# rare-resilience-ai/Osteosarcoma_DiffusionModel

Hardware: AMD Instinct MI355X
Metric: synthetic patients/sec (full T-step reverse sample) (higher is better)
Workload: dtype f32; 1 GPU; reverse sampling of conditional patients, T=1000, D=2000 (50 mut + 1900 expr + 50 pathway), hidden [256,512,256], 3 scenario conditions (BASELINE config 3); patients_per_gpu=100000, T=1000, parallelism=patients sharded over 1 GPU(s), no collective, sampler=chain, chunk_rows=65536, streams=2, graph=True

## Files before the change

osteosarcoma_diffusionmodel_amd/csrc/chain.h:

```cpp
#pragma once
#include "gemm_glds.h"
#include "epilogues.h"
#include "xpose.h"
#include "launch.h"

namespace osd {

constexpr int CHAIN_MAX_LAYERS = 24;
enum : int { CK_INPUT = 0, CK_GN32 = 1, CK_GN64 = 2, CK_POST = 3 };
enum : unsigned { CHAIN_OK = 0, CHAIN_TIMEOUT = 1, CHAIN_ABORT = 2 };

struct ChainLayer {
  const float* A; int lda;
  int K, K0;
  int F;
  int in0, ld0, in1, ld1;
  int out, ldo;
  int kind;
  const float* bias; const float* gamma; const float* beta;
};

struct ChainArgs {
  ChainLayer L[CHAIN_MAX_LAYERS];
  int n_layers;
  float* ws; long long ws_stride;
  float* x; int D;
  int n, n_tiles;
  int t_first, n_steps;
  unsigned base_done;
  const float* cproj; int ldc;
  const float* temb; int ldt;
  const float* coef;
  const float* z; int ldzz; long long z_step_stride; int z_t_first;
  uint64_t seed; uint32_t row_offset;
  float* mut_mask; int mutation_dim;
  unsigned* progress;
  unsigned* status;
  unsigned* queue;
  unsigned* cu_arrivals;
  int stagger;
  unsigned long long spin_budget;
  unsigned long long* stamps;
};

typedef __attribute__((address_space(1))) unsigned gu32;

__device__ __forceinline__ unsigned ld_relaxed_agent(const unsigned* p) {
  return __hip_atomic_load(p, __ATOMIC_RELAXED, __HIP_MEMORY_SCOPE_AGENT);
}
__device__ __forceinline__ void st_relaxed_agent(unsigned* p, unsigned v) {
  __hip_atomic_store(p, v, __ATOMIC_RELAXED, __HIP_MEMORY_SCOPE_AGENT);
}

__device__ __forceinline__ bool chain_wait(const unsigned* word, unsigned want, unsigned* status, unsigned long long budget, int lane) {
  if ((unsigned)__builtin_amdgcn_readfirstlane((int)ld_relaxed_agent(word)) >= want) return true;
  const unsigned long long t0 = __builtin_amdgcn_s_memrealtime();
  for (;;) {
    __builtin_amdgcn_s_sleep(32);
    if ((unsigned)__builtin_amdgcn_readfirstlane((int)ld_relaxed_agent(word)) >= want) return true;
    if ((unsigned)__builtin_amdgcn_readfirstlane((int)ld_relaxed_agent(status)) != CHAIN_OK) return false;
    if (__builtin_amdgcn_s_memrealtime() - t0 > budget) {
      if (lane == 0) st_relaxed_agent(status, CHAIN_TIMEOUT);
      return false;
    }
  }
}

constexpr int CHAIN_PRM_FLOATS = 512;

template <int NPB>
struct XposeRowsOut {
  const WaveXpose<NPB>& xp; float* out; int ldo;
  __device__ __forceinline__ void put(int fb, int pb, int q, int l31, int h, float4 v) const { (void)fb; xp.put(pb, q, l31, h, v); }
  __device__ __forceinline__ void flush(int fb, int lane) const { xp.template store_rows<false>(out + 32 * fb, ldo, lane, 0, 0); }
};
template <int NPB>
struct XposeRowsIn {
  const WaveXpose<NPB>& xp; const float* src; int ld;
  __device__ __forceinline__ void load(int fb, int lane) const { xp.template load_rows<false>(src + 32 * fb, ld, lane, 0, 0); }
  __device__ __forceinline__ float4 get(int fb, int pb, int q, int l31, int h) const { (void)fb; return xp.get(pb, q, l31, h); }
};

template <int GW, int NFB, int NPB, int PS, class Out>
__device__ __forceinline__ void chain_gn_silu(f32x16 (&acc)[NFB][NPB], const float* __restrict__ prm, int fl, const Out& o, int lane,
                                              unsigned long long* ts = nullptr) {
  static_assert(GW >= 8 && NFB * 32 >= GW, "wave must own whole groups");
  constexpr int RPG = GW / 2;
  constexpr int NG = NFB * 16 / RPG;
  const int l31 = lane & 31, h = lane >> 5;
#pragma unroll
  for (int fb = 0; fb < NFB; ++fb)
#pragma unroll
    for (int q = 0; q < 4; ++q) {
      const float4 bv = *reinterpret_cast<const float4*>(prm + fl + 32 * fb + 8 * q + 4 * h);
#pragma unroll
      for (int pb = 0; pb < NPB; ++pb) {
        acc[fb][pb][4 * q] += bv.x; acc[fb][pb][4 * q + 1] += bv.y;
        acc[fb][pb][4 * q + 2] += bv.z; acc[fb][pb][4 * q + 3] += bv.w;
      }
    }
  if (ts) { asm volatile("s_waitcnt vmcnt(0) lgkmcnt(0)" ::: "memory"); ts[0] = __builtin_amdgcn_s_memtime(); }
  float mean[NPB][NG], rstd[NPB][NG];
#pragma unroll
  for (int pb = 0; pb < NPB; ++pb)
#pragma unroll
    for (int g = 0; g < NG; ++g) {
      float s = 0.f;
#pragma unroll
      for (int j = 0; j < RPG; ++j) { const int Li = g * RPG + j; s += acc[Li / 16][pb][Li % 16]; }
      s += swap_halves(s);
      const float m = s * (1.0f / GW);
      float qs = 0.f;
#pragma unroll
      for (int j = 0; j < RPG; ++j) { const int Li = g * RPG + j; const float d = acc[Li / 16][pb][Li % 16] - m; qs = fmaf(d, d, qs); }
      qs += swap_halves(qs);
      mean[pb][g] = m;
      rstd[pb][g] = 1.0f / sqrtf(qs * (1.0f / GW) + GN_EPS);
    }
  if (ts) { asm volatile("s_nop 0" ::: "memory"); ts[1] = __builtin_amdgcn_s_memtime(); ts[2] = ts[1]; }
#pragma unroll
  for (int fb = 0; fb < NFB; ++fb) {
#pragma unroll
    for (int q = 0; q < 4; ++q) {
      const int f = fl + 32 * fb + 8 * q + 4 * h;
      const float4 gv = *reinterpret_cast<const float4*>(prm + PS + f);
      const float4 bev = *reinterpret_cast<const float4*>(prm + 2 * PS + f);
      const int g = (fb * 16 + 4 * q) / RPG;
#pragma unroll
      for (int pb = 0; pb < NPB; ++pb) {
        const float m = mean[pb][g], r = rstd[pb][g];
        float4 y;
        y.x = silu_f(fmaf((acc[fb][pb][4 * q] - m) * r, gv.x, bev.x));
        y.y = silu_f(fmaf((acc[fb][pb][4 * q + 1] - m) * r, gv.y, bev.y));
        y.z = silu_f(fmaf((acc[fb][pb][4 * q + 2] - m) * r, gv.z, bev.z));
        y.w = silu_f(fmaf((acc[fb][pb][4 * q + 3] - m) * r, gv.w, bev.w));
        o.put(fb, pb, q, l31, h, y);
      }
    }
    o.flush(fb, lane);
  }
}

template <int NFB, int NPB, int PS, class In, class Out>
__device__ __forceinline__ void chain_input(f32x16 (&acc)[NFB][NPB], const float* __restrict__ prm, int fl, const In& in, const Out& o, int lane) {
  const int l31 = lane & 31, h = lane >> 5;
#pragma unroll
  for (int fb = 0; fb < NFB; ++fb) {
    in.load(fb, lane);
#pragma unroll
    for (int q = 0; q < 4; ++q) {
      const int f = fl + 32 * fb + 8 * q + 4 * h;
      const float4 bv = *reinterpret_cast<const float4*>(prm + f);
      const float4 tv = *reinterpret_cast<const float4*>(prm + PS + f);
#pragma unroll
      for (int pb = 0; pb < NPB; ++pb) {
        const float4 cv = in.get(fb, pb, q, l31, h);
        float4 v;
        v.x = ((acc[fb][pb][4 * q] + bv.x) + tv.x) + cv.x;
        v.y = ((acc[fb][pb][4 * q + 1] + bv.y) + tv.y) + cv.y;
        v.z = ((acc[fb][pb][4 * q + 2] + bv.z) + tv.z) + cv.z;
        v.w = ((acc[fb][pb][4 * q + 3] + bv.w) + tv.w) + cv.w;
        o.put(fb, pb, q, l31, h, v);
      }
    }
    o.flush(fb, lane);
  }
}

#ifndef OSD_EXP
#define OSD_EXP 0
#endif
template <int NFB, int NPB, bool PRE = false, bool GUARD = true>
__device__ __forceinline__ void chain_posterior(f32x16 (&acc)[NFB][NPB], const float* __restrict__ prm, int fl, float* __restrict__ x, int ldx,
                                                int prow, int pcol, float cA, float cB, float cC, int t, const float* __restrict__ zrow, int ldzz,
                                                uint64_t seed, uint32_t row_id0, int f_glob, float* __restrict__ mut_mask, int mutation_dim,
                                                const WaveXpose<NPB>& xp, int lane, float4 (*pre)[4 * NPB] = nullptr) {
  const int l31 = lane & 31, h = lane >> 5;
  if (prow <= 0) return;
  const bool do_mask = t == 0 && mut_mask != nullptr;
#pragma unroll
  for (int fb = 0; fb < NFB; ++fb) {
    const int cols = pcol - 32 * fb;
    if (GUARD && cols <= 0) break;
    if constexpr (PRE) {
      if (!(OSD_EXP & 2)) {
        xp.commit_rows(*pre, lane);
        if (fb + 1 < NFB && cols - 32 > 0) xp.template issue_rows<GUARD>(*pre, x + 32 * (fb + 1), ldx, lane, prow, cols - 32);
      }
    } else {
      xp.template load_rows<GUARD>(x + 32 * fb, ldx, lane, prow, cols);
    }
#pragma unroll
    for (int pb = 0; pb < NPB; ++pb) {
      const int p = 32 * pb + l31;
      const int pc = (!GUARD || p < prow) ? p : prow - 1;
#pragma unroll
      for (int q = 0; q < 4; ++q) {
        const int fo = 32 * fb + 8 * q + 4 * h;
        const float4 bv = *reinterpret_cast<const float4*>(prm + fl + fo);
        const float e[4] = {acc[fb][pb][4 * q] + bv.x, acc[fb][pb][4 * q + 1] + bv.y, acc[fb][pb][4 * q + 2] + bv.z, acc[fb][pb][4 * q + 3] + bv.w};
        const float4 xq = xp.get(pb, q, l31, h);
        const float xv[4] = {xq.x, xq.y, xq.z, xq.w};
        float4 zz = make_float4(0.f, 0.f, 0.f, 0.f);
        if (t > 0 && cC != 0.f) {
          if (zrow) {
            const int fc = (!GUARD || fo < pcol - 4) ? fo : pcol - 4;
            zz = ldg4(zrow + (size_t)pc * ldzz + fc);
          } else if (!(OSD_EXP & 1)) {
            zz = randn4(seed, row_id0 + (uint32_t)p, (uint32_t)((f_glob + fo) >> 2), (uint32_t)t, TAG_POSTERIOR);
          }
        }
        const float zv[4] = {zz.x, zz.y, zz.z, zz.w};
        float o[4];
#pragma unroll
        for (int r = 0; r < 4; ++r) o[r] = fmaf(cA, xv[r], fmaf(cB, e[r], cC * zv[r]));
        if (do_mask && p < prow && fo < pcol && f_glob + fo < mutation_dim) {
          float* mrow = mut_mask + (size_t)p * mutation_dim;
#pragma unroll
          for (int r = 0; r < 4; ++r)
            if (f_glob + fo + r < mutation_dim) stg1(mrow + f_glob + fo + r, (o[r] > 0.5f) ? 1.0f : 0.0f);
        }
        xp.put(pb, q, l31, h, make_float4(o[0], o[1], o[2], o[3]));
      }
    }
    if (!(OSD_EXP & 4)) xp.template store_rows<GUARD>(x + 32 * fb, ldx, lane, prow, cols);
  }
}

#ifndef CHAIN_EPI_PRIO
#define CHAIN_EPI_PRIO 0
#endif
#ifndef CHAIN_BP
#define CHAIN_BP 128
#endif
#if CHAIN_BP == 128
typedef Tile<128, 128, 64, 64> ChainTile;
constexpr int CHAIN_WPS = 2;
#else
typedef Tile<128, 64, 64, 32> ChainTile;
constexpr int CHAIN_WPS = 3;
#endif
#ifdef OSD_DIAG
constexpr int CHAIN_KCNT = 12;
constexpr int CHAIN_STAMP_FLOATS = 2 * 4 * CHAIN_KCNT;
#else
constexpr int CHAIN_KCNT = 10;
constexpr int CHAIN_STAMP_FLOATS = 80;
#endif
constexpr int CHAIN_PRM_OFF = 2 * (ChainTile::BF * BK + ChainTile::BP * BK) + 4 + CHAIN_STAMP_FLOATS;
constexpr int CHAIN_LDS_BYTES = (CHAIN_PRM_OFF + 2 * CHAIN_PRM_FLOATS) * 4;
static_assert(CHAIN_PRM_OFF % 4 == 0, "parameter blocks are read as float4");

template <bool STAMP>
__global__ __launch_bounds__(NTHREADS, CHAIN_WPS) void chain_kernel(const ChainArgs* __restrict__ gp) {
  const ChainArgs& a = *gp;
  typedef ChainTile T;
  typedef GldsTile<T> G;
  static_assert(T::BF == 128 && T::BP % 32 == 0, "staging below assumes a 128-row weight image");
  constexpr int NW = NTHREADS / 64;
  constexpr int NPW = 16 / NW;
  constexpr int NPWB = T::BP / 8 / NW;
  constexpr int PROWS = 8 * NW;
  constexpr unsigned PBYTES = 1024u * NW;
  extern __shared__ __attribute__((aligned(16))) float smem[];
  float* As0 = smem;
  float* As1 = smem + G::A_ELEMS;
  float* Bs0 = smem + 2 * G::A_ELEMS;
  float* Bs1 = smem + 2 * G::A_ELEMS + G::B_ELEMS;
  volatile int& s_flag = *reinterpret_cast<volatile int*>(smem + 2 * (G::A_ELEMS + G::B_ELEMS));

  const int tid = threadIdx.x;
  const int lane = tid & 63;
  const int wave = __builtin_amdgcn_readfirstlane(tid >> 6);
  const int wf = (wave / T::NWP) * T::WF;
  const int wp = (wave % T::NWP) * T::WP;

  float* const ws = a.ws + (long long)blockIdx.x * a.ws_stride;
  WaveXpose<T::NPB> xp;
  {
    const int xo = wave * (T::NPB * 1024);
    xp.buf = xo < G::A_ELEMS ? As1 + xo : Bs1 + (xo - G::A_ELEMS);
  }
  float* const prm_base = smem + CHAIN_PRM_OFF;
  int pcur = 0;

  if (a.cu_arrivals && a.stagger > 0) {
    if (wave == 0) {
      const unsigned hw = __builtin_amdgcn_s_getreg(0xF804);
      const unsigned xcc = __builtin_amdgcn_s_getreg(0xF814) & 7;
      const unsigned key = (xcc << 8) | ((hw >> 8) & 0xFF);
      unsigned r = 0;
      if (lane == 0) r = atomicAdd(a.cu_arrivals + key, 1u);
      s_flag = __builtin_amdgcn_readfirstlane((int)(r & 1u));
    }
    __syncthreads();
    const int late = __builtin_amdgcn_readfirstlane(s_flag);
    __syncthreads();
    if (late) {
      const unsigned long long t0 = __builtin_amdgcn_s_memtime();
      while (__builtin_amdgcn_s_memtime() - t0 < (unsigned long long)a.stagger) __builtin_amdgcn_s_sleep(16);
    }
  }

  unsigned long long c_dep = 0, c_pro = 0, c_k = 0, c_epi = 0, c_units = 0;
  unsigned long long* const kcnt = reinterpret_cast<unsigned long long*>(smem + 2 * (G::A_ELEMS + G::B_ELEMS) + 4);
  if constexpr (STAMP) {
    if (tid < 4 * CHAIN_KCNT) kcnt[tid] = 0;
    __syncthreads();
  }
  const unsigned long long c_start = STAMP ? __builtin_amdgcn_s_memtime() : 0;
  const long long n_units = (long long)a.n_tiles * a.n_steps;
  int c_iter = 0;
  (void)c_iter;
  for (;;) {
    const unsigned long long td0 = STAMP ? __builtin_amdgcn_s_memtime() : 0;
#ifdef CHAIN_STATIC_UNITS
    static_assert(true, "");
    const long long u = (long long)blockIdx.x + (long long)c_iter * gridDim.x;
    ++c_iter;
#else
    if (wave == 0) {
      unsigned nu = 0;
      if (lane == 0) nu = atomicAdd(a.queue, 1u);
      s_flag = __builtin_amdgcn_readfirstlane((int)nu);
    }
    __syncthreads();
    const long long u = (unsigned)__builtin_amdgcn_readfirstlane(s_flag);
    __syncthreads();
#endif
    if (u >= n_units) break;
    const int tile = (int)(u % a.n_tiles);
    const int si = (int)(u / a.n_tiles);
    const int t = a.t_first - si;
    const int p0 = tile * T::BP;
    const int P = (a.n - p0 < T::BP) ? a.n - p0 : T::BP;

    if (wave == 0) {
      bool ok = (unsigned)__builtin_amdgcn_readfirstlane((int)ld_relaxed_agent(a.status)) == CHAIN_OK;
      if (ok && si > 0) {
        ok = chain_wait(a.progress + tile, a.base_done + (unsigned)si, a.status, a.spin_budget, lane);
        if (ok) __builtin_amdgcn_fence(__ATOMIC_ACQUIRE, "agent");
      }
      s_flag = ok ? 1 : 0;
      asm volatile("s_waitcnt vmcnt(0) lgkmcnt(0)" ::: "memory");
    }
    __syncthreads();
    const int go = __builtin_amdgcn_readfirstlane(s_flag);
    if (!go) return;
    if constexpr (STAMP) { c_dep += __builtin_amdgcn_s_memtime() - td0; ++c_units; }

    auto first_stage = [&](const ChainLayer& Lr, int f0n, bool do_a, bool do_b, int pb) {
      struct { const float* A; int lda, F, in0, ld0, K0, K; } Ln{Lr.A, Lr.lda, Lr.F, Lr.in0, Lr.ld0, Lr.K0, Lr.K};
      if (do_a && wave < 2) {
        const int kind = Lr.kind;
        const float* src = Lr.bias;
        if (wave == 1) src = Lr.beta;
        else if (lane >= 32) src = kind == CK_INPUT ? a.temb + (size_t)t * a.ldt : (kind == CK_POST ? Lr.bias : Lr.gamma);
        if (wave == 0 || (kind != CK_INPUT && kind != CK_POST)) {
          int f = f0n + 4 * (lane & 31);
          f = f < Ln.F - 4 ? f : Ln.F - 4;
          glds16(src + f, __builtin_amdgcn_readfirstlane(lds_addr(prm_base + pb * CHAIN_PRM_FLOATS) + (unsigned)wave * 1024u));
        }
      }
      const float* const xrows = a.x + (size_t)p0 * a.D;
      int ln = lane;
      asm volatile("" : "+v"(ln));
      const int r0 = wave * 8 + (ln >> 3);
      const int k4 = 4 * ((ln & 7) ^ ((r0 >> 1) & 7));
      const unsigned la = __builtin_amdgcn_readfirstlane(lds_addr(As0) + (unsigned)wave * 1024u);
      const unsigned lb = __builtin_amdgcn_readfirstlane(lds_addr(Bs0) + (unsigned)wave * 1024u);
      if (do_a) {
#pragma unroll
        for (int j = 0; j < NPW; ++j) {
          int rg = f0n + r0 + PROWS * j;
          rg = rg < Ln.F ? rg : Ln.F - 1;
          glds16(Ln.A + (size_t)rg * Ln.lda + k4, __builtin_amdgcn_readfirstlane(la + (unsigned)j * PBYTES));
        }
      }
      if (do_b) {
        const bool from_x = Ln.in0 < 0;
        const float* bb = from_x ? xrows : ws + Ln.in0;
        const int rows = from_x ? P : T::BP;
        const int kend = Ln.K0 < Ln.K ? Ln.K0 : Ln.K;
        const int k = k4 < kend - 4 ? k4 : kend - 4;
#pragma unroll
        for (int j = 0; j < NPWB; ++j) {
          int rg = r0 + PROWS * j;
          rg = rg < rows ? rg : rows - 1;
          glds16(bb + (size_t)rg * Ln.ld0 + k, __builtin_amdgcn_readfirstlane(lb + (unsigned)j * PBYTES));
        }
      }
    };
    unsigned long long tt0 = STAMP ? __builtin_amdgcn_s_memtime() : 0;
    first_stage(a.L[0], 0, true, true, pcur);
    asm volatile("s_waitcnt vmcnt(0)" ::: "memory");
    __syncthreads();

    for (int l = 0; l < a.n_layers; ++l) {
      const ChainLayer& L = a.L[l];
      const gfloat_ptr LA = uniform_ptr(L.A);
      const int Llda = L.lda, LK0 = L.K0, Lld0 = L.ld0, Lld1 = L.ld1;
      const int F = L.F, K = L.K;
      const float* const B0g = (L.in0 < 0) ? a.x + (size_t)p0 * a.D : ws + L.in0;
      const float* const B1g = ws + L.in1;
      const gfloat_ptr B0 = uniform_ptr(B0g), B1 = uniform_ptr(B1g);
      const int rowsB = (L.in0 < 0) ? P : T::BP;
      const int nk = (K + BK - 1) / BK;
      const int nft = (F + T::BF - 1) / T::BF;
      for (int ft = 0; ft < nft; ++ft) {
        const int f0 = ft * T::BF;
        int ln = lane;
        asm volatile("" : "+v"(ln));
        const int l31 = ln & 31, h = ln >> 5;
        int st_row[NPW], st_k4[NPW];
#pragma unroll
        for (int j = 0; j < NPW; ++j) {
          st_row[j] = (j * NW + wave) * 8 + (ln >> 3);
          st_k4[j] = 4 * ((ln & 7) ^ ((st_row[j] >> 1) & 7));
        }
        int a_rd[T::NFB], a_sw[T::NFB], b_rd[T::NPB], b_sw[T::NPB];
#pragma unroll
        for (int fb = 0; fb < T::NFB; ++fb) { const int R = wf + 32 * fb + l31; a_rd[fb] = R * BK; a_sw[fb] = h ^ ((R >> 1) & 7); }
#pragma unroll
        for (int pb = 0; pb < T::NPB; ++pb) { const int R = wp + 32 * pb + l31; b_rd[pb] = R * BK; b_sw[pb] = h ^ ((R >> 1) & 7); }
        unsigned offA[NPW], offB[NPWB];
#pragma unroll
        for (int j = 0; j < NPW; ++j) {
          int rg = f0 + st_row[j];
          rg = rg < F ? rg : F - 1;
          offA[j] = (unsigned)(rg * Llda + st_k4[j]) * 4u;
        }
#pragma unroll
        for (int j = 0; j < NPWB; ++j) {
          int rb = st_row[j];
          rb = rb < rowsB ? rb : rowsB - 1;
          offB[j] = (unsigned)(rb * Lld0 + st_k4[j]) * 4u;
        }
        int b_panel = 0;
        auto b_offsets_for = [&](int k0) {
          const int want = k0 < LK0 ? 0 : 1;
          if (want != b_panel) {
            b_panel = want;
            const int ld = want ? Lld1 : Lld0;
#pragma unroll
            for (int j = 0; j < NPWB; ++j) {
              int rb = st_row[j];
              rb = rb < rowsB ? rb : rowsB - 1;
              offB[j] = (unsigned)(rb * ld + st_k4[j]) * 4u;
            }
          }
        };
        struct StageCtx { gfloat_ptr sa, sb; unsigned la, lb; int k0; bool tail; };
        auto stage_begin = [&](int k0, float* As, float* Bs) {
          b_offsets_for(k0);
          const bool first = k0 < LK0;
          const int kend = first ? (LK0 < K ? LK0 : K) : K - LK0;
          const int kl = first ? k0 : k0 - LK0;
          StageCtx c;
          c.sa = LA + __builtin_amdgcn_readfirstlane(k0);
          c.sb = (first ? B0 : B1) + __builtin_amdgcn_readfirstlane(kl);
          c.la = __builtin_amdgcn_readfirstlane(lds_addr(As) + (unsigned)wave * 1024u);
          c.lb = __builtin_amdgcn_readfirstlane(lds_addr(Bs) + (unsigned)wave * 1024u);
          c.k0 = k0;
          c.tail = kl + BK > kend;
          return c;
        };
        auto piece = [&](const StageCtx& c, int j) {
          if (j < NPW) glds16s(c.sa, offA[j], __builtin_amdgcn_readfirstlane(c.la + (unsigned)j * PBYTES));
          else glds16s(c.sb, offB[j - NPW], __builtin_amdgcn_readfirstlane(c.lb + (unsigned)(j - NPW) * PBYTES));
        };
        auto stage_tail = [&](const StageCtx& c) {
#pragma unroll
          for (int j = 0; j < NPW; ++j) piece(c, j);
          const bool first = c.k0 < LK0;
          const int kend = first ? (LK0 < K ? LK0 : K) : K - LK0;
          const int kl = first ? c.k0 : c.k0 - LK0;
          const float* bb = first ? B0g : B1g;
          const int ld = first ? Lld0 : Lld1;
#pragma unroll
          for (int jb = 0; jb < NPWB; ++jb) {
            int k = kl + st_k4[jb];
            k = k < kend - 4 ? k : kend - 4;
            int rg = st_row[jb];
            rg = rg < rowsB ? rg : rowsB - 1;
            glds16(bb + (size_t)rg * ld + k, __builtin_amdgcn_readfirstlane(c.lb + (unsigned)jb * PBYTES));
          }
        };
        const unsigned long long tt1 = STAMP ? __builtin_amdgcn_s_memtime() : 0;

        unsigned long long c_kw = 0, c_kb = 0;
        (void)c_kw; (void)c_kb;
        f32x16 acc[T::NFB][T::NPB];
#pragma unroll
        for (int i = 0; i < T::NFB; ++i)
#pragma unroll
          for (int j = 0; j < T::NPB; ++j)
#pragma unroll
            for (int r = 0; r < 16; ++r) acc[i][j][r] = 0.f;

        float fa0[T::NFB][4], fb0[T::NPB][4], fa1[T::NFB][4], fb1[T::NPB][4];
        auto frags = [&](const float* Ac, const float* Bc, int i, float (&fa)[T::NFB][4], float (&fb)[T::NPB][4]) {
#pragma unroll
          for (int fb_ = 0; fb_ < T::NFB; ++fb_) {
            const float4 tq = *reinterpret_cast<const float4*>(&Ac[a_rd[fb_] + 4 * (a_sw[fb_] ^ (2 * i))]);
            fa[fb_][0] = tq.x; fa[fb_][1] = tq.y; fa[fb_][2] = tq.z; fa[fb_][3] = tq.w;
          }
#pragma unroll
          for (int pb = 0; pb < T::NPB; ++pb) {
            const float4 tq = *reinterpret_cast<const float4*>(&Bc[b_rd[pb] + 4 * (b_sw[pb] ^ (2 * i))]);
            fb[pb][0] = tq.x; fb[pb][1] = tq.y; fb[pb][2] = tq.z; fb[pb][3] = tq.w;
          }
        };
        auto quarter = [&](const float (&fa)[T::NFB][4], const float (&fb)[T::NPB][4]) {
#pragma unroll
          for (int e = 0; e < 4; ++e)
#pragma unroll
            for (int fb_ = 0; fb_ < T::NFB; ++fb_)
#pragma unroll
              for (int pb = 0; pb < T::NPB; ++pb)
                acc[fb_][pb] = __builtin_amdgcn_mfma_f32_32x32x2f32(fa[fb_][e], fb[pb][e], acc[fb_][pb], 0, 0, 0);
        };
        __builtin_amdgcn_sched_barrier(0);
        if (nk > 1) {
          const StageCtx c = stage_begin(BK, As1, Bs1);
          if (c.tail) stage_tail(c);
          else {
#pragma unroll
            for (int j = 0; j < NPW + NPWB; ++j) piece(c, j);
          }
        }
        frags(As0, Bs0, 0, fa0, fb0);
        __builtin_amdgcn_sched_barrier(0);
        for (int kt = 0; kt < nk; ++kt) {
          float* Ac = (kt & 1) ? As1 : As0;
          float* Bc = (kt & 1) ? Bs1 : Bs0;
          const float* An = (kt & 1) ? As0 : As1;
          const float* Bn = (kt & 1) ? Bs0 : Bs1;
          frags(Ac, Bc, 1, fa1, fb1);
          quarter(fa0, fb0);
          frags(Ac, Bc, 2, fa0, fb0);
          quarter(fa1, fb1);
          frags(Ac, Bc, 3, fa1, fb1);
          const bool ahead = kt + 2 < nk;
          StageCtx c{};
          if (ahead) c = stage_begin((kt + 2) * BK, Ac, Bc);
          const bool whole = ahead && !c.tail;
          quarter(fa0, fb0);
          __builtin_amdgcn_sched_barrier(0);
          const unsigned long long tw0 = STAMP ? __builtin_amdgcn_s_memtime() : 0;
          asm volatile("s_waitcnt vmcnt(0)" ::: "memory");
          const unsigned long long tw1 = STAMP ? __builtin_amdgcn_s_memtime() : 0;
          asm volatile("s_waitcnt lgkmcnt(0)" ::: "memory");
          __syncthreads();
          if constexpr (STAMP) { const unsigned long long tw2 = __builtin_amdgcn_s_memtime(); c_kw += tw1 - tw0; c_kb += tw2 - tw1; }
          __builtin_amdgcn_sched_barrier(0);
          if (ahead && c.tail) stage_tail(c);
          if (whole) {
#pragma unroll
            for (int j = 0; j < NPW + NPWB; ++j) piece(c, j);
          }
          if (kt + 1 < nk) frags(An, Bn, 0, fa0, fb0);
          __builtin_amdgcn_sched_barrier(0);
          quarter(fa1, fb1);
        }

        const unsigned long long tt2 = STAMP ? __builtin_amdgcn_s_memtime() : 0;
        const bool same_layer = ft + 1 < nft;
        const bool has_next = same_layer || l + 1 < a.n_layers;
        const int ln_next = same_layer ? l : l + 1;
        const int f0_next = same_layer ? f0 + T::BF : 0;
        const bool early_b = same_layer;
        if (has_next) first_stage(a.L[ln_next], f0_next, true, early_b, pcur ^ 1);
        const int fw = f0 + wf;
        const float* const prm = prm_base + pcur * CHAIN_PRM_FLOATS;
        pcur ^= 1;
        if (CHAIN_EPI_PRIO) __builtin_amdgcn_s_setprio(CHAIN_EPI_PRIO);
        const ChainArgs* ep = gp;
        asm volatile("" : "+s"(ep));
        const ChainArgs& e = *ep;
        unsigned long long ets[3] = {0, 0, 0};
        if (L.kind == CK_GN64) {
          const XposeRowsOut<T::NPB> o{xp, ws + L.out + (size_t)wp * L.ldo + fw, L.ldo};
          chain_gn_silu<64, T::NFB, T::NPB, 128>(acc, prm, wf, o, lane, STAMP ? ets : nullptr);
        } else if (L.kind == CK_GN32) {
          const XposeRowsOut<T::NPB> o{xp, ws + L.out + (size_t)wp * L.ldo + fw, L.ldo};
          chain_gn_silu<32, T::NFB, T::NPB, 128>(acc, prm, wf, o, lane, STAMP ? ets : nullptr);
        } else if (L.kind == CK_INPUT) {
          const XposeRowsIn<T::NPB> ci{xp, e.cproj + (size_t)(p0 + wp) * e.ldc + fw, e.ldc};
          const XposeRowsOut<T::NPB> o{xp, ws + L.out + (size_t)wp * L.ldo + fw, L.ldo};
          chain_input<T::NFB, T::NPB, 128>(acc, prm, wf, ci, o, lane);
        } else {
          const float* c = e.coef + 4 * t;
          const float cA = c[0], cB = c[1], cC = c[2];
          const float* zrow = e.z ? e.z + (long long)(e.z_t_first - t) * e.z_step_stride + (size_t)(p0 + wp) * e.ldzz + fw : nullptr;
          float* const mm = e.mut_mask ? e.mut_mask + (size_t)(p0 + wp) * e.mutation_dim : nullptr;
          chain_posterior<T::NFB, T::NPB>(acc, prm, wf, e.x + (size_t)(p0 + wp) * e.D + fw, e.D, P - wp, F - fw, cA, cB, cC, t, zrow, e.ldzz,
                                          e.seed, e.row_offset + (uint32_t)(p0 + wp), fw, mm, e.mutation_dim, xp, lane);
        }
        if (CHAIN_EPI_PRIO) __builtin_amdgcn_s_setprio(0);
        unsigned long long tt3 = 0, te1 = 0, te2 = 0, te3 = 0, te4 = 0;
        if constexpr (STAMP) te1 = __builtin_amdgcn_s_memtime();
        if (early_b) {
          if constexpr (STAMP) tt3 = __builtin_amdgcn_s_memtime();
          static_assert(4 * T::NFB * T::NPB == 16 || 4 * T::NFB * T::NPB == 8, "counted wait below is written for 16 or 8 stores");
          if (L.kind == CK_POST) asm volatile("s_waitcnt vmcnt(0)" ::: "memory");
          else if (4 * T::NFB * T::NPB == 16) asm volatile("s_waitcnt vmcnt(16)" ::: "memory");
          else asm volatile("s_waitcnt vmcnt(8)" ::: "memory");
          if constexpr (STAMP) te2 = __builtin_amdgcn_s_memtime();
          __syncthreads();
          if constexpr (STAMP) te3 = te4 = __builtin_amdgcn_s_memtime();
        } else {
          asm volatile("s_waitcnt vmcnt(0)" ::: "memory");
          if constexpr (STAMP) te2 = __builtin_amdgcn_s_memtime();
          __syncthreads();
          if constexpr (STAMP) tt3 = te3 = __builtin_amdgcn_s_memtime();
          if (has_next) {
            first_stage(a.L[ln_next], 0, false, true, 0);
            asm volatile("s_waitcnt vmcnt(0)" ::: "memory");
            __syncthreads();
          }
          if constexpr (STAMP) te4 = __builtin_amdgcn_s_memtime();
        }
        if constexpr (STAMP) {
          c_pro += tt1 - tt0; c_k += tt2 - tt1; c_epi += tt3 - tt2;
          tt0 = tt3;
          if (tid == 0) {
            unsigned long long* kc = kcnt + CHAIN_KCNT * L.kind;
            kc[0] += tt2 - tt1; kc[1] += te1 - tt2; kc[2] += te2 - te1; kc[3] += te3 - te2; kc[4] += te4 - te3; kc[5] += 1;
            if constexpr (CHAIN_KCNT >= 12) { kc[10] += c_kw; kc[11] += c_kb; }
            if (ets[0]) { kc[6] += ets[0] - tt2; kc[7] += ets[1] - ets[0]; kc[8] += ets[2] - ets[1]; kc[9] += te1 - ets[2]; }
          }
        }
      }
    }

    if (wave == 0) {
      __builtin_amdgcn_fence(__ATOMIC_RELEASE, "agent");
      asm volatile("s_waitcnt vmcnt(0)" ::: "memory");
      if (lane == 0) st_relaxed_agent(a.progress + tile, a.base_done + (unsigned)si + 1u);
    }
  }
  if (STAMP && a.stamps && tid == 0) {
    unsigned long long* o = a.stamps + (size_t)blockIdx.x * 64;
    o[0] = c_dep; o[1] = c_pro; o[2] = c_k; o[3] = c_epi; o[4] = __builtin_amdgcn_s_memtime() - c_start; o[5] = c_units;
    o[6] = __builtin_amdgcn_s_getreg(0xF804);
    o[7] = __builtin_amdgcn_s_getreg(0xF814) & 7;
    for (int i = 0; i < 4 * CHAIN_KCNT; ++i) o[8 + i] = kcnt[i];
  }
}

}
```

osteosarcoma_diffusionmodel_amd/csrc/gemm_glds.h:

```cpp
#pragma once
#include "gemm.h"

namespace osd {

typedef __attribute__((address_space(3))) void* lds_ptr_t;
typedef const __attribute__((address_space(1))) void* glb_ptr_t;

__device__ __forceinline__ void glds16(const float* gsrc, unsigned lds_dst) {
  unsigned keep;
  asm volatile(
      "s_mov_b32 %0, m0\n\t"
      "s_mov_b32 m0, %2\n\t"
      "s_nop 0\n\t"
      "global_load_lds_dwordx4 %1, off\n\t"
      "s_mov_b32 m0, %0"
      : "=&s"(keep)
      : "v"(gsrc), "s"(lds_dst)
      : "memory");
}
typedef const __attribute__((address_space(1))) float* gfloat_ptr;
__device__ __forceinline__ gfloat_ptr uniform_ptr(const float* p) {
  const gfloat_ptr q = (gfloat_ptr)p;
  const unsigned long long v = reinterpret_cast<unsigned long long>(q);
  const unsigned lo = __builtin_amdgcn_readfirstlane((unsigned)v), hi = __builtin_amdgcn_readfirstlane((unsigned)(v >> 32));
  return reinterpret_cast<gfloat_ptr>(((unsigned long long)hi << 32) | lo);
}
__device__ __forceinline__ void glds16s(gfloat_ptr sbase, unsigned voff, unsigned lds_dst) {
  unsigned keep;
  asm volatile(
      "s_mov_b32 %0, m0\n\t"
      "s_mov_b32 m0, %3\n\t"
      "s_nop 4\n\t"
      "global_load_lds_dwordx4 %1, %2\n\t"
      "s_mov_b32 m0, %0"
      : "=&s"(keep)
      : "v"(voff), "s"(sbase), "s"(lds_dst)
      : "memory");
}
__device__ __forceinline__ unsigned lds_addr(const float* p) {
  return (unsigned)(uintptr_t)(__attribute__((address_space(3))) const void*)p;
}

template <class T>
struct GldsTile {
  static constexpr int A_ELEMS = T::BF * BK;
  static constexpr int B_ELEMS = T::BP * BK;
  static constexpr int LDS_BYTES = 2 * (A_ELEMS + B_ELEMS) * 4;
  static constexpr int NA = T::BF / 32;
  static constexpr int NB = T::BP / 32;
};

template <class T, class Epi, int NG = 1>
__global__ __launch_bounds__(NTHREADS * NG, NG == 1 ? 2 : 1) void gemm_glds_kernel(GemmArgs g, typename Epi::Args ea) {
  typedef GldsTile<T> G;
  static_assert(NG == 1 || NG == 2, "one or two wave groups");
  extern __shared__ __attribute__((aligned(16))) float smem_all[];
  const int grp = NG == 1 ? 0 : __builtin_amdgcn_readfirstlane((int)(threadIdx.x >> 8));
  float* const smem = smem_all + grp * (G::LDS_BYTES / 4);
  float* As0 = smem;
  float* As1 = smem + G::A_ELEMS;
  float* Bs0 = smem + 2 * G::A_ELEMS;
  float* Bs1 = smem + 2 * G::A_ELEMS + G::B_ELEMS;

  const int nft = (g.F + T::BF - 1) / T::BF;
  const int npt = (g.P + T::BP - 1) / T::BP;
  const int b = blockIdx.x;
  const int idx = b >> 3;
  const int ft = idx % nft;
  int pt, pstride;
  if (g.persist) {
    const int per_xcd = gridDim.x >> 3;
    pt = idx / nft + (per_xcd / nft) * (b & 7);
    pstride = gridDim.x / nft;
  } else {
    pt = (idx / nft) * 8 + (b & 7);
    pstride = npt;
  }
  if (pt >= npt) return;
  if (g.tri && ft > pt) return;
  const int f0 = ft * T::BF;

  const int tid = threadIdx.x & (NTHREADS - 1);
  const int lane = tid & 63;
  const int wave = __builtin_amdgcn_readfirstlane(tid >> 6);
  unsigned long long st0 = 0, st1 = 0, st2 = 0;
  if (g.stamps) st0 = __builtin_amdgcn_s_memtime();
  const int wf = (wave / T::NWP) * T::WF;
  const int wp = (wave % T::NWP) * T::WP;
  const int l31 = lane & 31, h = lane >> 5;

  const auto pre = Epi::template prefetch<T::NFB, true>(ea, f0 + wf, lane, g.F);

  int a_off[G::NA], a_k4[G::NA];
  int b_k4[G::NB], b_lrow[G::NB];
#pragma unroll
  for (int j = 0; j < G::NA; ++j) {
    const int row = (j * 4 + wave) * 8 + (lane >> 3);
    int rg = f0 + row;
    rg = rg < g.F ? rg : g.F - 1;
    a_k4[j] = 4 * ((lane & 7) ^ ((row >> 1) & 7));
    a_off[j] = rg * g.lda + a_k4[j];
  }
#pragma unroll
  for (int j = 0; j < G::NB; ++j) {
    const int row = (j * 4 + wave) * 8 + (lane >> 3);
    b_lrow[j] = row;
    b_k4[j] = 4 * ((lane & 7) ^ ((row >> 1) & 7));
  }
  struct StageCtx { unsigned la, lb; const float* bbase; int bld, bk, bkend, ak, p0; };
  auto stage_begin = [&](int k0, int p0, float* As, float* Bs) {
    StageCtx c;
    c.la = __builtin_amdgcn_readfirstlane(lds_addr(As) + (unsigned)wave * 1024u);
    c.lb = __builtin_amdgcn_readfirstlane(lds_addr(Bs) + (unsigned)wave * 1024u);
    const bool first = k0 < g.K0;
    c.bbase = first ? g.B0 : g.B1;
    c.bld = first ? g.ldb0 : g.ldb1;
    c.bk = first ? k0 : k0 - g.K0;
    c.bkend = first ? (g.K0 < g.K ? g.K0 : g.K) : g.K - g.K0;
    c.ak = k0;
    c.p0 = p0;
    return c;
  };
  auto stage_piece = [&](const StageCtx& c, int j) {
    if (j < G::NA) {
      int adj = 0;
      if (g.a_kmax > 0) {
        const int k = c.ak + a_k4[j];
        adj = k < g.a_kmax - 4 ? 0 : g.a_kmax - 4 - k;
      }
      glds16(g.A + (size_t)(a_off[j] + c.ak + adj), __builtin_amdgcn_readfirstlane(c.la + (unsigned)j * 4096u));
    } else {
      const int jb = j - G::NA;
      int k = c.bk + b_k4[jb];
      k = k < c.bkend - 4 ? k : c.bkend - 4;
      int rg = c.p0 + b_lrow[jb];
      rg = rg < g.P ? rg : g.P - 1;
      glds16(c.bbase + (size_t)rg * c.bld + k, __builtin_amdgcn_readfirstlane(c.lb + (unsigned)jb * 4096u));
    }
  };
  constexpr int NPIECE = G::NA + G::NB;

  int a_rd[T::NFB], a_sw[T::NFB], b_rd[T::NPB], b_sw[T::NPB];
#pragma unroll
  for (int fb = 0; fb < T::NFB; ++fb) { const int R = wf + 32 * fb + l31; a_rd[fb] = R * BK; a_sw[fb] = h ^ ((R >> 1) & 7); }
#pragma unroll
  for (int pb = 0; pb < T::NPB; ++pb) { const int R = wp + 32 * pb + l31; b_rd[pb] = R * BK; b_sw[pb] = h ^ ((R >> 1) & 7); }

  f32x16 acc[T::NFB][T::NPB];

  auto compute = [&](const float* As, const float* Bs, int i, const StageCtx& sc, bool do_stage) {
    float a[T::NFB][4], bb[T::NPB][4];
#pragma unroll
    for (int fb = 0; fb < T::NFB; ++fb) {
      const float4 t = *reinterpret_cast<const float4*>(&As[a_rd[fb] + 4 * (a_sw[fb] ^ (2 * i))]);
      a[fb][0] = t.x; a[fb][1] = t.y; a[fb][2] = t.z; a[fb][3] = t.w;
    }
#pragma unroll
    for (int pb = 0; pb < T::NPB; ++pb) {
      const float4 t = *reinterpret_cast<const float4*>(&Bs[b_rd[pb] + 4 * (b_sw[pb] ^ (2 * i))]);
      bb[pb][0] = t.x; bb[pb][1] = t.y; bb[pb][2] = t.z; bb[pb][3] = t.w;
    }
#pragma unroll
    for (int e = 0; e < 4; ++e) {
#pragma unroll
      for (int fb = 0; fb < T::NFB; ++fb)
#pragma unroll
        for (int pb = 0; pb < T::NPB; ++pb)
          acc[fb][pb] = __builtin_amdgcn_mfma_f32_32x32x2f32(a[fb][e], bb[pb][e], acc[fb][pb], 0, 0, 0);
      if (do_stage && i == 0) {
        __builtin_amdgcn_sched_barrier(0);
        if (2 * e < NPIECE) stage_piece(sc, 2 * e);
        if (2 * e + 1 < NPIECE) stage_piece(sc, 2 * e + 1);
        __builtin_amdgcn_sched_barrier(0);
      }
    }
  };

  const int nk_all = (g.K + BK - 1) / BK;
  const int nk = NG == 1 ? nk_all : (nk_all + 1) / 2;
  const int kbeg = grp ? nk : 0;
  const int kcnt = NG == 1 ? nk : (grp ? nk_all - nk : nk);
  {
    const StageCtx c0 = stage_begin(kbeg * BK, pt * T::BP, As0, Bs0);
#pragma unroll
    for (int j = 0; j < NPIECE; ++j) stage_piece(c0, j);
  }
  constexpr int FULL_TILE_STORES = T::NFB * T::NPB * 4;
  bool counted_wait = false;
  for (; pt < npt; pt += pstride) {
    const int p0 = pt * T::BP;
    if (counted_wait) {
      if constexpr (FULL_TILE_STORES == 16) asm volatile("s_waitcnt vmcnt(16)" ::: "memory");
      else if constexpr (FULL_TILE_STORES == 8) asm volatile("s_waitcnt vmcnt(8)" ::: "memory");
      else if constexpr (FULL_TILE_STORES == 4) asm volatile("s_waitcnt vmcnt(4)" ::: "memory");
      else asm volatile("s_waitcnt vmcnt(0)" ::: "memory");
    } else {
      asm volatile("s_waitcnt vmcnt(0)" ::: "memory");
    }
    __syncthreads();
    if (g.stamps && st1 == 0) st1 = __builtin_amdgcn_s_memtime();
#pragma unroll
    for (int i = 0; i < T::NFB; ++i)
#pragma unroll
      for (int j = 0; j < T::NPB; ++j)
#pragma unroll
        for (int r = 0; r < 16; ++r) acc[i][j][r] = 0.f;
    for (int kt = 0; kt < nk; ++kt) {
      float* Ac = (kt & 1) ? As1 : As0;
      float* Bc = (kt & 1) ? Bs1 : Bs0;
      const bool more = kt + 1 < kcnt;
      const StageCtx sc = stage_begin(more ? (kbeg + kt + 1) * BK : 0, p0, (kt & 1) ? As0 : As1, (kt & 1) ? Bs0 : Bs1);
      if (NG == 1 || kt < kcnt) {
        compute(Ac, Bc, 0, sc, more);
        compute(Ac, Bc, 1, sc, more);
        compute(Ac, Bc, 2, sc, more);
        compute(Ac, Bc, 3, sc, more);
      }
      asm volatile("s_waitcnt vmcnt(0)" ::: "memory");
      __syncthreads();
    }
    if (g.stamps && st2 == 0) st2 = __builtin_amdgcn_s_memtime();
    const int ptn = pt + pstride;
    if (ptn < npt) {
      const StageCtx cn = stage_begin(0, ptn * T::BP, As0, Bs0);
#pragma unroll
      for (int j = 0; j < NPIECE; ++j) stage_piece(cn, j);
    }
    if constexpr (NG == 2) {
      constexpr int NREG = T::NFB * T::NPB * 16;
      static_assert(4 * NREG * 64 * 4 <= G::LDS_BYTES, "accumulator hand-over must fit the group's staging buffers");
      float* const red = smem_all + G::LDS_BYTES / 4 + wave * (NREG * 64);
      if (grp == 1) {
#pragma unroll
        for (int i = 0; i < T::NFB; ++i)
#pragma unroll
          for (int j = 0; j < T::NPB; ++j)
#pragma unroll
            for (int r = 0; r < 16; ++r) red[((i * T::NPB + j) * 16 + r) * 64 + lane] = acc[i][j][r];
      }
      __syncthreads();
      if (grp == 1) return;
#pragma unroll
      for (int i = 0; i < T::NFB; ++i)
#pragma unroll
        for (int j = 0; j < T::NPB; ++j)
#pragma unroll
          for (int r = 0; r < 16; ++r) acc[i][j][r] += red[((i * T::NPB + j) * 16 + r) * 64 + lane];
    }
    counted_wait = Epi::COUNTED_STORES && (p0 + T::BP <= g.P) && (f0 + T::BF <= g.F);
    if constexpr (Epi::XBUF) {
      constexpr int XR = T::NPB * 1024;
      static_assert(G::A_ELEMS % XR == 0 && 4 * XR <= G::A_ELEMS + G::B_ELEMS, "transposer regions must tile the idle buffers");
      const int xo = wave * XR;
      float* const xb = xo < G::A_ELEMS ? As1 + xo : Bs1 + (xo - G::A_ELEMS);
      Epi::template apply<T::NFB, T::NPB, true>(acc, ea, pre, f0 + wf, p0 + wp, lane, g.F, g.P, xb);
    } else {
      Epi::template apply<T::NFB, T::NPB, true>(acc, ea, pre, f0 + wf, p0 + wp, lane, g.F, g.P);
    }
  }
  if (g.stamps) {
    asm volatile("s_waitcnt vmcnt(0)" ::: "memory");
    const unsigned long long st3 = __builtin_amdgcn_s_memtime();
    if (lane == 0) {
      unsigned long long* o = g.stamps + ((size_t)blockIdx.x * 4 + wave) * 4;
      o[0] = st0; o[1] = st1; o[2] = st2; o[3] = st3;
    }
  }
}

}
```

Measured before the change: 23060 patients/s.

## Unroll chain k-loop by buffer parity and precompute LDS fragment addresses

```diff
diff --git a/osteosarcoma_diffusionmodel_amd/csrc/chain.h b/osteosarcoma_diffusionmodel_amd/csrc/chain.h
--- a/osteosarcoma_diffusionmodel_amd/csrc/chain.h
+++ b/osteosarcoma_diffusionmodel_amd/csrc/chain.h
@@ -1,4 +1,5 @@
 #pragma once
+#include <type_traits>
 #include "gemm_glds.h"
 #include "epilogues.h"
 #include "xpose.h"
@@ -418,11 +419,15 @@
           st_row[j] = (j * NW + wave) * 8 + (ln >> 3);
           st_k4[j] = 4 * ((ln & 7) ^ ((st_row[j] >> 1) & 7));
         }
-        int a_rd[T::NFB], a_sw[T::NFB], b_rd[T::NPB], b_sw[T::NPB];
-#pragma unroll
-        for (int fb = 0; fb < T::NFB; ++fb) { const int R = wf + 32 * fb + l31; a_rd[fb] = R * BK; a_sw[fb] = h ^ ((R >> 1) & 7); }
-#pragma unroll
-        for (int pb = 0; pb < T::NPB; ++pb) { const int R = wp + 32 * pb + l31; b_rd[pb] = R * BK; b_sw[pb] = h ^ ((R >> 1) & 7); }
+        static_assert(T::WF % 32 == 0 && T::WP % 32 == 0, "the swizzle term must not depend on the wave's first row");
+        unsigned fr_a[4], fr_b[4];
+#pragma unroll
+        for (int i = 0; i < 4; ++i) {
+          const unsigned chunk = 16u * (unsigned)((h ^ ((l31 >> 1) & 7)) ^ (2 * i));
+          fr_a[i] = lds_addr(As0) + (unsigned)(wf + l31) * (BK * 4u) + chunk;
+          fr_b[i] = lds_addr(Bs0) + (unsigned)(wp + l31) * (BK * 4u) + chunk;
+          asm volatile("" : "+v"(fr_a[i]), "+v"(fr_b[i]));
+        }
         unsigned offA[NPW], offB[NPWB];
 #pragma unroll
         for (int j = 0; j < NPW; ++j) {
@@ -436,17 +441,14 @@
           rb = rb < rowsB ? rb : rowsB - 1;
           offB[j] = (unsigned)(rb * Lld0 + st_k4[j]) * 4u;
         }
-        int b_panel = 0;
+        const int k_switch = __builtin_amdgcn_readfirstlane(LK0 < K ? LK0 / BK : nk);
         auto b_offsets_for = [&](int k0) {
-          const int want = k0 < LK0 ? 0 : 1;
-          if (want != b_panel) {
-            b_panel = want;
-            const int ld = want ? Lld1 : Lld0;
+          if (__builtin_amdgcn_readfirstlane(k0) == k_switch * BK) {
 #pragma unroll
             for (int j = 0; j < NPWB; ++j) {
               int rb = st_row[j];
               rb = rb < rowsB ? rb : rowsB - 1;
-              offB[j] = (unsigned)(rb * ld + st_k4[j]) * 4u;
+              offB[j] = (unsigned)(rb * Lld1 + st_k4[j]) * 4u;
             }
           }
         };
@@ -469,6 +471,10 @@
           if (j < NPW) glds16s(c.sa, offA[j], __builtin_amdgcn_readfirstlane(c.la + (unsigned)j * PBYTES));
           else glds16s(c.sb, offB[j - NPW], __builtin_amdgcn_readfirstlane(c.lb + (unsigned)(j - NPW) * PBYTES));
         };
+        auto stage_whole = [&](const StageCtx& c) {
+          static_assert(NPW == 4, "glds16s_stage moves four weight pieces");
+          glds16s_stage<NPWB, PBYTES>(c.sa, c.sb, c.la, c.lb, offA, offB);
+        };
         auto stage_tail = [&](const StageCtx& c) {
 #pragma unroll
           for (int j = 0; j < NPW; ++j) piece(c, j);
@@ -499,15 +505,18 @@
             for (int r = 0; r < 16; ++r) acc[i][j][r] = 0.f;
 
         float fa0[T::NFB][4], fb0[T::NPB][4], fa1[T::NFB][4], fb1[T::NPB][4];
-        auto frags = [&](const float* Ac, const float* Bc, int i, float (&fa)[T::NFB][4], float (&fb)[T::NPB][4]) {
+        typedef float lds_f32x4 __attribute__((ext_vector_type(4)));
+        typedef const __attribute__((address_space(3))) lds_f32x4* lds_f32x4_ptr;
+        auto frags = [&](auto parc, int i, float (&fa)[T::NFB][4], float (&fb)[T::NPB][4]) {
+          constexpr int PAR = decltype(parc)::value;
 #pragma unroll
           for (int fb_ = 0; fb_ < T::NFB; ++fb_) {
-            const float4 tq = *reinterpret_cast<const float4*>(&Ac[a_rd[fb_] + 4 * (a_sw[fb_] ^ (2 * i))]);
+            const lds_f32x4 tq = *(lds_f32x4_ptr)(uintptr_t)(fr_a[i] + (unsigned)(PAR * G::A_ELEMS * 4 + fb_ * 32 * BK * 4));
             fa[fb_][0] = tq.x; fa[fb_][1] = tq.y; fa[fb_][2] = tq.z; fa[fb_][3] = tq.w;
           }
 #pragma unroll
           for (int pb = 0; pb < T::NPB; ++pb) {
-            const float4 tq = *reinterpret_cast<const float4*>(&Bc[b_rd[pb] + 4 * (b_sw[pb] ^ (2 * i))]);
+            const lds_f32x4 tq = *(lds_f32x4_ptr)(uintptr_t)(fr_b[i] + (unsigned)(PAR * G::B_ELEMS * 4 + pb * 32 * BK * 4));
             fb[pb][0] = tq.x; fb[pb][1] = tq.y; fb[pb][2] = tq.z; fb[pb][3] = tq.w;
           }
         };
@@ -524,24 +533,24 @@
         if (nk > 1) {
           const StageCtx c = stage_begin(BK, As1, Bs1);
           if (c.tail) stage_tail(c);
-          else {
-#pragma unroll
-            for (int j = 0; j < NPW + NPWB; ++j) piece(c, j);
-          }
-        }
-        frags(As0, Bs0, 0, fa0, fb0);
+          else stage_whole(c);
+        }
+        constexpr std::integral_constant<int, 0> buf0{};
+        constexpr std::integral_constant<int, 1> buf1{};
+        frags(buf0, 0, fa0, fb0);
         __builtin_amdgcn_sched_barrier(0);
-        for (int kt = 0; kt < nk; ++kt) {
-          float* Ac = (kt & 1) ? As1 : As0;
-          float* Bc = (kt & 1) ? Bs1 : Bs0;
-          const float* An = (kt & 1) ? As0 : As1;
-          const float* Bn = (kt & 1) ? Bs0 : Bs1;
-          frags(Ac, Bc, 1, fa1, fb1);
+        auto kstep = [&](auto parc, auto lastc, int kt) {
+          constexpr int PAR = decltype(parc)::value;
+          constexpr bool LAST = decltype(lastc)::value;
+          constexpr std::integral_constant<int, PAR ^ 1> nextc{};
+          float* const Ac = PAR ? As1 : As0;
+          float* const Bc = PAR ? Bs1 : Bs0;
+          frags(parc, 1, fa1, fb1);
           quarter(fa0, fb0);
-          frags(Ac, Bc, 2, fa0, fb0);
+          frags(parc, 2, fa0, fb0);
           quarter(fa1, fb1);
-          frags(Ac, Bc, 3, fa1, fb1);
-          const bool ahead = kt + 2 < nk;
+          frags(parc, 3, fa1, fb1);
+          const bool ahead = !LAST && kt + 2 < nk;
           StageCtx c{};
           if (ahead) c = stage_begin((kt + 2) * BK, Ac, Bc);
           const bool whole = ahead && !c.tail;
@@ -555,13 +564,20 @@
           if constexpr (STAMP) { const unsigned long long tw2 = __builtin_amdgcn_s_memtime(); c_kw += tw1 - tw0; c_kb += tw2 - tw1; }
           __builtin_amdgcn_sched_barrier(0);
           if (ahead && c.tail) stage_tail(c);
-          if (whole) {
-#pragma unroll
-            for (int j = 0; j < NPW + NPWB; ++j) piece(c, j);
-          }
-          if (kt + 1 < nk) frags(An, Bn, 0, fa0, fb0);
+          if (whole) stage_whole(c);
+          if (!LAST && kt + 1 < nk) frags(nextc, 0, fa0, fb0);
           __builtin_amdgcn_sched_barrier(0);
           quarter(fa1, fb1);
+        };
+        {
+          constexpr std::false_type more{};
+          constexpr std::true_type last{};
+          int kt = 0;
+          for (; kt + 1 < nk; kt += 2) {
+            kstep(buf0, more, kt);
+            kstep(buf1, more, kt + 1);
+          }
+          if (kt < nk) kstep(buf0, last, kt);
         }
 
         const unsigned long long tt2 = STAMP ? __builtin_amdgcn_s_memtime() : 0;
diff --git a/osteosarcoma_diffusionmodel_amd/csrc/gemm_glds.h b/osteosarcoma_diffusionmodel_amd/csrc/gemm_glds.h
--- a/osteosarcoma_diffusionmodel_amd/csrc/gemm_glds.h
+++ b/osteosarcoma_diffusionmodel_amd/csrc/gemm_glds.h
@@ -37,6 +37,36 @@
       : "v"(voff), "s"(sbase), "s"(lds_dst)
       : "memory");
 }
+#define OSD_GLDS_P0(LD, V, S) "s_mov_b32 m0, " LD "\n\ts_nop 0\n\tglobal_load_lds_dwordx4 " V ", " S "\n\t"
+#define OSD_GLDS_PJ(LD, O, V, S) "s_add_u32 m0, " LD ", " O "\n\ts_nop 0\n\tglobal_load_lds_dwordx4 " V ", " S "\n\t"
+template <int NB, unsigned PB>
+__device__ __forceinline__ void glds16s_stage(gfloat_ptr sa, gfloat_ptr sb, unsigned la, unsigned lb, const unsigned (&va)[4],
+                                              const unsigned (&vb)[NB]) {
+  static_assert(NB == 2 || NB == 4, "two or four activation pieces per wave");
+  unsigned keep;
+  if constexpr (NB == 4)
+    asm volatile(
+        "s_mov_b32 %0, m0\n\t"
+        OSD_GLDS_P0("%3", "%5", "%1") OSD_GLDS_PJ("%3", "%13", "%6", "%1") OSD_GLDS_PJ("%3", "%14", "%7", "%1") OSD_GLDS_PJ("%3", "%15", "%8", "%1")
+        OSD_GLDS_P0("%4", "%9", "%2") OSD_GLDS_PJ("%4", "%13", "%10", "%2") OSD_GLDS_PJ("%4", "%14", "%11", "%2") OSD_GLDS_PJ("%4", "%15", "%12", "%2")
+        "s_mov_b32 m0, %0"
+        : "=&s"(keep)
+        : "s"(sa), "s"(sb), "s"(la), "s"(lb), "v"(va[0]), "v"(va[1]), "v"(va[2]), "v"(va[3]), "v"(vb[0]), "v"(vb[1]), "v"(vb[2]), "v"(vb[3]),
+          "i"(PB), "i"(2 * PB), "i"(3 * PB)
+        : "memory", "scc");
+  else
+    asm volatile(
+        "s_mov_b32 %0, m0\n\t"
+        OSD_GLDS_P0("%3", "%5", "%1") OSD_GLDS_PJ("%3", "%11", "%6", "%1") OSD_GLDS_PJ("%3", "%12", "%7", "%1") OSD_GLDS_PJ("%3", "%13", "%8", "%1")
+        OSD_GLDS_P0("%4", "%9", "%2") OSD_GLDS_PJ("%4", "%11", "%10", "%2")
+        "s_mov_b32 m0, %0"
+        : "=&s"(keep)
+        : "s"(sa), "s"(sb), "s"(la), "s"(lb), "v"(va[0]), "v"(va[1]), "v"(va[2]), "v"(va[3]), "v"(vb[0]), "v"(vb[1]),
+          "i"(PB), "i"(2 * PB), "i"(3 * PB)
+        : "memory", "scc");
+}
+#undef OSD_GLDS_P0
+#undef OSD_GLDS_PJ
 __device__ __forceinline__ unsigned lds_addr(const float* p) {
   return (unsigned)(uintptr_t)(__attribute__((address_space(3))) const void*)p;
 }
```

Measured after the change: 23180 patients/s, median of 6. No clear change (+0.5%).
